# Shinzef/BlenderRayTracer

Hardware: AMD Instinct MI355X
Metric: Msamples/s (pixels×spp/s) at 1/2/4/8 MI355X; % HBM roofline; RMS vs JS ref (higher is better)
Workload: dtype f64; 1 GPU; config3_rtow_1920x1080_512spp; scene=rtow.json, width=1920, height=1080, spp=512, max_depth=5, primitives=486, accel=auto, parallelism=1 GPU

## Files before the change

__graft_entry__.py:

```python
import os
import sys

ROOT = os.path.dirname(os.path.abspath(__file__))
if ROOT not in sys.path:
    sys.path.insert(0, ROOT)


def build() -> None:
    from blenderraytracer_amd import build as b
    b.build_lib(force=True)
    b.build_cli(force=True)
    b.build_napi(force=True)
    from oracle import binding
    binding.build()
    sys.path.insert(0, os.path.join(ROOT, "tests"))
    import hostcheck_binding
    hostcheck_binding.build()
    hostcheck_binding.lib(("RT_HOST_COUNTERS=1",))
    import texcheck_binding
    texcheck_binding.build()
    import lightcheck_binding
    lightcheck_binding.build()
    import guidedcheck_binding
    guidedcheck_binding.build()
    import neecheck_binding
    for mutation in (0, 1, 2):
        neecheck_binding.build(mutation)
    import blenderraytracer_amd
    from blenderraytracer_amd import capi
    capi.load_library()


def smoke() -> None:
    import numpy as np

    from blenderraytracer_amd import capi
    from blenderraytracer_amd.renderer import GpuRayTracer
    from blenderraytracer_amd.scene import load_scene_json
    from oracle import binding

    rt = GpuRayTracer(64, 48, seed=7, device=0, precision=capi.RT_PREC_F64)
    assert rt.load_from_json(load_scene_json("sample_scene.json"))
    rt.update_render_settings({"maxBounces": 4, "samples": 4})
    r = rt.render(want=("mean", "segments"))
    o = binding.render(rt.packed(), rt.settings())
    assert np.array_equal(r["segments"], o["segments"]), "segment counts differ from the oracle"
    err = np.max(np.abs(r["mean"] - o["mean"]))
    assert err <= 1e-12, f"GPU vs oracle max abs diff {err}"
    assert np.array_equal(r["rgba8"], o["rgba8"])
    print(f"smoke ok: 64x48x4spp sample_scene, {rt.last_stats.kernel_ms:.3f} ms kernel, max|diff| {err:.1e}")
    rt.close()
    rt = GpuRayTracer(48, 27, seed=7, device=0, precision=capi.RT_PREC_F64)
    assert rt.load_from_json(load_scene_json("rtow.json"))
    rt.update_render_settings({"maxBounces": 5, "samples": 4})
    lib = capi.load_library()
    assert lib.rt_scene_walk(rt.scene_handle(), capi.RT_PREC_F64, capi.RT_ACCEL_AUTO) == 2, "RTOW should walk the grid"
    r = rt.render(want=("mean", "segments"))
    o = binding.render(rt.packed(), rt.settings())
    assert np.array_equal(r["segments"], o["segments"]), "RTOW segment counts differ from the oracle"
    err = np.max(np.abs(r["mean"] - o["mean"]))
# ... 11 lines not shown
```

blenderraytracer_amd/csrc/pt_core.h:

```cpp
#pragma once
#include <hip/hip_runtime.h>
#include <math.h>
#include <stdint.h>
#include <string.h>
#include "js_math.h"

#define RT_HD __host__ __device__ __forceinline__
#ifndef RT_COLD_BG
#define RT_COLD_BG 1
#endif
#if RT_COLD_BG && defined(__HIP_DEVICE_COMPILE__)
#define RT_COLD __attribute__((noinline))
#else
#define RT_COLD
#endif
#define RT_COLD_HD __host__ __device__ RT_COLD

namespace rt {

template <class R> RT_HD R js_pow(R x, R y) {
    if constexpr (sizeof(R) == 8) return jsm::pow(x, y);
    else return pow(x, y);
}
template <class R> RT_HD R js_exp(R x) {
// ... 107 lines not shown
    if (div_rcp_on<R>() && min3abs(a) >= xmin && l >= smin && l <= smax)
        return {div_rcp_1(a.x, l, y), div_rcp_1(a.y, l, y), div_rcp_1(a.z, l, y)};
    return vdiv(a, l);
}
template <class R> RT_HD V3<R> normalize(V3<R> a) {
    R l = sqrt(a.x * a.x + a.y * a.y + a.z * a.z);
#if RT_DIV_RCP
    return l > (R)0 ? vdiv_rcp_unit(a, l, (R)1 / l) : mk<R>(0, 0, 0);
#else
    return l > (R)0 ? vdiv(a, l) : mk<R>(0, 0, 0);
#endif
}
template <class R> RT_HD V3<R> reflect(V3<R> a, V3<R> n) {
    return a - n * ((R)2 * dot(a, n));
}

enum RunKind : int { RUN_SPHERES = 0, RUN_PLANES = 1, RUN_BOXES = 2, RUN_TRIANGLES = 3, RUN_MESH = 4 };
struct Run { int kind, begin, end, mat; };

template <class R> struct SphereRec { R cx, cy, cz, r2; };
struct SphereFilter { float cx, cy, cz, r2p; };
#ifndef RT_FILTER_MARGIN
#define RT_FILTER_MARGIN (-17)
#endif
constexpr double filter_margin() {
    double v = 1.0;
    for (int k = 0; k > RT_FILTER_MARGIN; --k) v *= 0.5;
    return v;
}
template <class R> struct PlaneRec { R px, py, pz, nx, ny, nz; };
template <class R> struct BoxRec { R mnx, mny, mnz, mxx, mxy, mxz; };
template <class R> struct TriRec { R v0x, v0y, v0z, e1x, e1y, e1z, e2x, e2y, e2z, nx, ny, nz; };
template <class R> struct MatRec { int type, pad; R c[3]; R p; };
template <class R> struct SphereLeaf { SphereFilter f; SphereRec<R> s; int id, obj, mat, pad; };
template <> struct SphereLeaf<float> { SphereRec<float> s; int id, obj, mat, pad; };
template <class R> struct TriGeom { R v0x, v0y, v0z, e1x, e1y, e1z, e2x, e2y, e2z; };
template <class R> struct alignas(16) TriLeaf { TriGeom<R> t; int id, obj; };
struct alignas(16) TriFilter { float v0[3], e1[3], e2[3], n[3]; };

struct BvhNode { float lo[3]; int skip; float hi[3]; int fc; };
struct Bvh2Node { float lo[3][2]; float hi[3][2]; int child[2]; int pad[2]; };
#ifndef RT_BVH_STACK
#define RT_BVH_STACK 24
#endif

enum TexType : int { TEX_CHECKER = 0, TEX_NOISE = 1, TEX_MARBLE = 2, TEX_WOOD = 3 };
template <class R> struct TexRec { int type, perm; R scale; R odd[3], even[3]; };
template <class R> struct TexView { const TexRec<R>* recs; const int* perms; const int* mat_tex; int num, num_perms; };
enum LightType : int { LIGHT_POINT = 0, LIGHT_DIRECTIONAL = 1 };
template <class R> struct LightRec { int type, pad; R v[3]; R color[3]; R intensity; };
template <class R> struct LightView { const LightRec<R>* recs; int num, pad; };
enum EmitterKind : int { EMIT_SPHERE = 0, EMIT_TRI = 1 };
template <class R> struct EmitterRec { int kind, idx; R g[12]; R le[3]; R area; };
template <class R> struct EmitterView { const EmitterRec<R>* recs; const int* sphere_listed; const R* tri_area; int num, pad; };

template <class R>
struct SceneView {
    const Run* runs;
    int num_runs;
    int num_prims;
    const SphereRec<R>* spheres;
    const SphereFilter* sphere_filter;
    int num_spheres;
    const R* sphere_r;
    const R* sphere_inv_r;
    const PlaneRec<R>* planes;
    const BoxRec<R>* boxes;
// ... 139 lines not shown
#if RT_FAST_RCP && defined(__HIP_DEVICE_COMPILE__)
    return __builtin_amdgcn_rcpf(x);
#else
    return 1.0f / x;
#endif
}
RT_HD float rt_rsqrt_approx(float x) {
#if RT_FAST_RCP && defined(__HIP_DEVICE_COMPILE__)
    return __builtin_amdgcn_rsqf(x);
#else
    return 1.0f / sqrtf(x);
#endif
}

struct FilterRay { float ox, oy, oz, dx, dy, dz, delta; };

template <class R>
RT_HD FilterRay make_filter_ray(V3<R> o, V3<R> d) {
    FilterRay f;
    f.ox = (float)o.x; f.oy = (float)o.y; f.oz = (float)o.z;
    const float dx = (float)d.x, dy = (float)d.y, dz = (float)d.z;
    const float inv = rt_rsqrt_approx(dx * dx + dy * dy + dz * dz);
    f.dx = dx * inv; f.dy = dy * inv; f.dz = dz * inv;
    f.delta = (f.ox * f.ox + f.oy * f.oy + f.oz * f.oz) * ((float)(2.0 * filter_margin()) * (1.0f + 0x1p-20f));
    return f;
}

RT_HD bool sphere_filter_pass(const SphereFilter& s, const FilterRay& r) {
    RT_HCOUNT(HC_FILTER_TESTS, 1);
    const float ocx = r.ox - s.cx, ocy = r.oy - s.cy, ocz = r.oz - s.cz;
    const float hb = __builtin_fmaf(ocx, r.dx, __builtin_fmaf(ocy, r.dy, ocz * r.dz));
    const float cc = __builtin_fmaf(ocx, ocx, __builtin_fmaf(ocy, ocy, __builtin_fmaf(ocz, ocz, -(s.r2p + r.delta))));
    return !(__builtin_fmaf(hb, hb, -cc) < 0.0f);
}

enum Feat : int { F_PLANES = 1, F_BOXES = 2, F_TRIS = 4, F_BGALL = 8, F_CAMALL = 16, F_ALL = 31,
                  F_TEX = 32,
                  F_LIGHT = 64,
                  F_NEE = 128 };

template <class R, int FEAT = F_ALL>
RT_HD Closest<R> closest_hit_runs(const SceneView<R>& sc, V3<R> o, V3<R> d) {
    const R tmin = (R)0.001;
    Closest<R> b{(R)INFINITY, HIT_NONE, 0, 0};
    const R a = dot(d, d);
    for (int r = 0; r < sc.num_runs; ++r) {
        const Run run = sc.runs[r];
        if (run.kind == RUN_SPHERES) {
            if constexpr (sizeof(R) == 8) {
                const FilterRay fr = make_filter_ray(o, d);
RT_UNROLL(RT_SPHERE_UNROLL)
                for (int i = run.begin; i < run.end; ++i) {
                    if (!sphere_filter_pass(sc.sphere_filter[i], fr)) continue;
                    sphere_test_f64(sc, o, d, a, tmin, i, b);
                }
                continue;
            }
#pragma unroll 2
            for (int i = run.begin; i < run.end; ++i) sphere_test_f64(sc, o, d, a, tmin, i, b);
        } else if ((FEAT & F_PLANES) != 0 && run.kind == RUN_PLANES) {
            for (int i = run.begin; i < run.end; ++i) {
                const PlaneRec<R> p = sc.planes[i];
                R denom = p.nx * d.x + p.ny * d.y + p.nz * d.z;
                if (fabs(denom) < (R)1e-6) continue;
                R t = ((p.px - o.x) * p.nx + (p.py - o.y) * p.ny + (p.pz - o.z) * p.nz) / denom;
                if (t < tmin || t > b.t) continue;
// ... 439 lines not shown
    const BvhRay br = make_bvh_ray(o, d);
    float tl = bvh_tlimit(b.t);
    if (sc.num_sphere_nodes > 0 || sc.num_big_spheres > 0) {
        const R a = dot(d, d);
        FilterRay fr{};
        if constexpr (sizeof(R) == 8) fr = make_filter_ray(o, d);
        if (sc.num_big_spheres > 0) sphere_records(sc.big_spheres, 0, sc.num_big_spheres, o, d, a, fr, tmin, b, tl, w, true);
        auto leaf = [&](int fc) { sphere_leaf(sc, fc, o, d, a, fr, tmin, b, tl, w); };
        if (sc.num_sphere_nodes > 0)
            bvh_walk<WIDE, LDSN ? 1 : 0>(sc.sphere_nodes, sc.num_sphere_nodes, sc.sphere_wide, br, tl, stk, w, leaf);
    }
    if (TRI && sc.num_tri_nodes > 0 && !skip_tri) {
        if constexpr (sizeof(R) == 8 && RT_TRI_FILTER != 0) {
            const TriRay tr = make_tri_ray(o, d);
            auto leaf = [&](int fc) { tri_leaf_filtered(sc, fc, tr, o, d, tmin, b, tl, w); };
            bvh_walk<WIDE, TLDS ? 2 : 0>(sc.tri_nodes, sc.num_tri_nodes, sc.tri_wide, br, tl, stk, w, leaf);
        } else {
            auto leaf = [&](int fc) { tri_leaf(sc, fc, o, d, tmin, b, tl, w); };
            bvh_walk<WIDE, TLDS ? 2 : 0>(sc.tri_nodes, sc.num_tri_nodes, sc.tri_wide, br, tl, stk, w, leaf);
        }
    }
    return b;
}

#ifndef RT_GRID_UNIFORM
#define RT_GRID_UNIFORM 2
#endif
#ifndef RT_GRID_DIV
#define RT_GRID_DIV 0
#endif
#ifndef RT_GRID_COMPACT
#define RT_GRID_COMPACT 1
#endif
template <class R>
RT_HD void sphere_records_lds(const rt_u4* lrec, const SphereLeaf<R>* recs, int first, int end, V3<R> o, V3<R> d,
                              R a, const FilterRay& fr, R tmin, Closest<R>& b, float& tl, Work& w, R ya = (R)0,
                              int origin = -1) {
    RT_COUNT(w.spheres += end - first);
    if constexpr (sizeof(R) == 8 && RT_GRID_COMPACT != 0) {
        for (int base = first; base < end; base += 32) {
            const int n = end - base < 32 ? end - base : 32;
            uint32_t pass = 0;
            for (int i = 0; i < n; ++i) {
                const rt_u4 q = lrec[base + i];
                SphereFilter f;
                memcpy(&f, &q, sizeof f);
                if (sphere_filter_pass(f, fr)) pass |= 1u << i;
            }
            while (pass) {
                const int k = base + __builtin_ctz(pass);
                pass &= pass - 1;
                const SphereRec<R> s = recs[k].s;
                const int id = recs[k].id, obj = recs[k].obj, mat = recs[k].mat;
                R t;
                if (!sphere_candidate(s, o, d, a, tmin, t, RT_ORIGIN_LEAVE && id == origin, ya)) continue;
                if (better(t, obj, id, b)) {
                    RT_HCOUNT(HC_ACCEPT, 1);
                    b = Closest<R>{t, HIT_SPHERE, id, mat, obj};
                    tl = bvh_tlimit(b.t);
                }
            }
        }
        return;
    }
    for (int k = first; k < end; ++k) {
        SphereRec<R> s;
        int id, obj, mat;
        if constexpr (sizeof(R) == 8) {
            const rt_u4 q = lrec[k];
            SphereFilter f;
            memcpy(&f, &q, sizeof f);
            if (!sphere_filter_pass(f, fr)) continue;
            s = recs[k].s;
            id = recs[k].id; obj = recs[k].obj; mat = recs[k].mat;
        } else {
            const rt_u4 q0 = lrec[2 * k], q1 = lrec[2 * k + 1];
            memcpy(&s, &q0, sizeof s);
            id = (int)q1.x; obj = (int)q1.y; mat = (int)q1.z;
        }
        R t;
        if (!sphere_candidate(s, o, d, a, tmin, t, false, ya)) continue;
        if (better(t, obj, id, b)) {
            RT_HCOUNT(HC_ACCEPT, 1);
            b = Closest<R>{t, HIT_SPHERE, id, mat, obj};
            tl = bvh_tlimit(b.t);
        }
    }
}

template <class R>
RT_HD size_t grid_lds_rec_bytes(const SceneView<R>& sc) { return (size_t)sc.num_grid_recs * (sizeof(R) == 8 ? 16 : 32); }
template <class R>
RT_HD size_t grid_lds_bytes(const SceneView<R>& sc) {
    return grid_lds_rec_bytes(sc) + 4 * (size_t)(sc.num_grid_cells + 1);
}
template <class R>
RT_HD void copy_grid_lds(const SceneView<R>& sc, rt_u4* grec, int* gcell, int t, int threads) {
    const rt_u4* g = reinterpret_cast<const rt_u4*>(sc.grid_leaf);
    for (int k = t; k < sc.num_grid_recs; k += threads) {
        if constexpr (sizeof(R) == 8) grec[k] = g[4 * k];
        else { grec[2 * k] = g[2 * k]; grec[2 * k + 1] = g[2 * k + 1]; }
    }
    for (int k = t; k <= sc.num_grid_cells; k += threads) gcell[k] = sc.grid_cell[k];
}

struct GridRefs { const int* n; const float *lo, *hi, *cs, *ics; float far; };

template <class R, bool LDSG = false, int FEAT = F_ALL, bool LOCAL = false>
RT_HD Closest<R> closest_hit_grid(const SceneView<R>& sc, V3<R> o, V3<R> d, Work& w, const BvhStack& stk, int origin = -1) {
    const R tmin = (R)0.001;
    Closest<R> b{(R)INFINITY, HIT_NONE, 0, 0, -1};
    brute_planes_boxes<R, FEAT>(sc, o, d, tmin, b);
    float tl = bvh_tlimit(b.t);
    const R a = dot(d, d), ya = root_rcp(a);
    FilterRay fr{};
    if constexpr (sizeof(R) == 8) fr = make_filter_ray(o, d);
    if (sc.num_big_spheres > 0) sphere_records(sc.big_spheres, 0, sc.num_big_spheres, o, d, a, fr, tmin, b, tl, w, true, ya);
    if (sc.num_grid_cells <= 0) return b;
    const GridRefs gp{sc.grid_n, sc.grid_lo, sc.grid_hi, sc.grid_cs, sc.grid_ics, sc.grid_far};
    auto at = [](const auto* a, int k) {
        if constexpr (LOCAL) return k == 0 ? a[0] : (k == 1 ? a[1] : a[2]);
        else return a[k];
    };
    const float of[3] = {(float)o.x, (float)o.y, (float)o.z};
    const float df[3] = {(float)d.x, (float)d.y, (float)d.z};
    if (!(fmaxf(fabsf(of[0]), fmaxf(fabsf(of[1]), fabsf(of[2]))) <= gp.far)) {
        sphere_records(sc.grid_leaf, 0, sc.grid_cell[sc.num_grid_cells], o, d, a, fr, tmin, b, tl, w);
        return b;
    }
    float inv[3], t0 = 0.0f, t1 = tl;
    for (int k = 0; k < 3; ++k) {
        float v = rt_rcp_approx(df[k]);
        if (!(fabsf(v) <= 0x1p126f)) v = copysignf(0x1p126f, df[k]);
        inv[k] = v;
        const float ta = (gp.lo[k] - of[k]) * v, tb = (gp.hi[k] - of[k]) * v;
        t0 = fmaxf(t0, fminf(ta, tb));
        t1 = fminf(t1, fmaxf(ta, tb));
    }
    if (!(t0 <= t1)) return b;
    int cell[3], step[3];
    float tmax[3];
    for (int k = 0; k < 3; ++k) {
        const float p = of[k] + t0 * df[k];
        const bool by_div = RT_GRID_DIV == 1 || (RT_GRID_DIV == 0 && sizeof(R) == 8);
        int c = by_div ? (int)floorf((p - gp.lo[k]) / gp.cs[k])
                       : (int)floorf((p - gp.lo[k]) * gp.ics[k]);
        c = c < 0 ? 0 : (c >= gp.n[k] ? gp.n[k] - 1 : c);
        cell[k] = c;
        step[k] = df[k] > 0.0f ? 1 : (df[k] < 0.0f ? -1 : 0);
        tmax[k] = step[k] == 0 ? INFINITY
                               : (gp.lo[k] + (float)(c + (step[k] > 0)) * gp.cs[k] - of[k]) * inv[k];
    }
    for (;;) {
        RT_COUNT(++w.nodes);
        const int ci = cell[0] + gp.n[0] * (cell[1] + gp.n[1] * cell[2]);
        if constexpr (LDSG) {
            sphere_records_lds(stk.grec, sc.grid_leaf, stk.gcell[ci], stk.gcell[ci + 1], o, d, a, fr, tmin, b, tl, w, ya, origin);
        } else {
#if RT_GRID_UNIFORM && defined(__HIP_DEVICE_COMPILE__)
        const int first = __builtin_amdgcn_readfirstlane(ci);
        if ((RT_GRID_UNIFORM == 1 || sizeof(R) == 4) && __ballot(ci != first) == 0)
            sphere_records(sc.grid_leaf, sc.grid_cell[first], sc.grid_cell[first + 1], o, d, a, fr, tmin, b, tl, w);
        else
#endif
        sphere_records(sc.grid_leaf, sc.grid_cell[ci], sc.grid_cell[ci + 1], o, d, a, fr, tmin, b, tl, w);
        }
        const int ax = tmax[0] <= tmax[1] ? (tmax[0] <= tmax[2] ? 0 : 2) : (tmax[1] <= tmax[2] ? 1 : 2);
        const float tx = tmax[ax];
        if (b.t < (R)tx || !(tx < INFINITY)) break;
        const int nc = cell[ax] + step[ax];
        if (nc < 0 || nc >= at(gp.n, ax)) break;
        cell[ax] = nc;
        tmax[ax] = (at(gp.lo, ax) + (float)(nc + (step[ax] > 0)) * at(gp.cs, ax) - of[ax]) * inv[ax];
    }
    return b;
}

enum Accel : int { ACC_BRUTE = 0, ACC_BRUTE_LEAN = 1, ACC_BVH = 2, ACC_BVH_STACK = 3, ACC_BVH_SPHERES = 4, ACC_BVH_SPHERES_LDS = 5,
                   ACC_GRID = 6, ACC_GRID_LDS = 7, ACC_BVH_TRI_LDS = 8, ACC_GRID_LDS_LEAN = 9,
                   ACC_BVH_STACK_LEAN = 10, ACC_BRUTE_TEX = 11, ACC_BVH_STACK_TEX = 12,
                   ACC_BRUTE_LIT = 13, ACC_BVH_STACK_LIT = 14, ACC_BRUTE_NEE = 15, ACC_BVH_STACK_NEE = 16 };
template <int ACC> constexpr int walk_of() {
    return ACC == ACC_BRUTE_TEX || ACC == ACC_BRUTE_LIT || ACC == ACC_BRUTE_NEE ? ACC_BRUTE
         : ACC == ACC_BVH_STACK_TEX || ACC == ACC_BVH_STACK_LIT || ACC == ACC_BVH_STACK_NEE ? ACC_BVH_STACK : ACC;
}
template <int ACC> constexpr int feat_of() {
    return ACC == ACC_GRID_LDS_LEAN ? 0 : ACC == ACC_BVH_STACK_LEAN ? (F_PLANES | F_TRIS)
         : ACC == ACC_BRUTE_LEAN ? F_PLANES : ACC == ACC_BRUTE_TEX || ACC == ACC_BVH_STACK_TEX ? (F_ALL | F_TEX)
         : ACC == ACC_BRUTE_LIT || ACC == ACC_BVH_STACK_LIT ? (F_ALL | F_TEX | F_LIGHT)
         : ACC == ACC_BRUTE_NEE || ACC == ACC_BVH_STACK_NEE ? (F_ALL | F_TEX | F_LIGHT | F_NEE) : F_ALL;
}

#ifndef RT_SC_RELOAD
#define RT_SC_RELOAD 2
#endif
template <class R, int ACC> constexpr bool sc_reload() {
    return sizeof(R) == 8 && (((RT_SC_RELOAD & 1) && ACC == ACC_BVH_STACK_LEAN) ||
                              ((RT_SC_RELOAD & 2) && ACC == ACC_GRID_LDS_LEAN) || ((RT_SC_RELOAD & 4) && ACC == ACC_BRUTE_LEAN));
}
template <class R, int ACC, bool LOCAL = false>
RT_HD Closest<R> closest_hit_acc(const SceneView<R>& sc, V3<R> o, V3<R> d, Work& w, BvhStack stk, bool skip_tri = false,
                                 int origin = -1) {
#if defined(__HIP_DEVICE_COMPILE__)
    if constexpr (!LOCAL && sc_reload<R, ACC>()) {
        typedef const __attribute__((address_space(4))) SceneView<R>* SvPtr;
        SvPtr p = (SvPtr)__builtin_amdgcn_kernarg_segment_ptr();
        asm volatile("" : "+s"(p));
        const SceneView<R> scl = *p;
        return closest_hit_acc<R, ACC, true>(scl, o, d, w, stk, skip_tri, origin);
    }
#endif
    if constexpr (walk_of<ACC>() != ACC) return closest_hit_acc<R, walk_of<ACC>(), LOCAL>(sc, o, d, w, stk, skip_tri, origin);
    else if constexpr (ACC == ACC_BVH) return closest_hit_bvh<R, false>(sc, o, d, w, stk, skip_tri);
    else if constexpr (ACC == ACC_BVH_STACK) return closest_hit_bvh<R, true>(sc, o, d, w, stk, skip_tri);
    else if constexpr (ACC == ACC_BVH_SPHERES) return closest_hit_bvh<R, true, false>(sc, o, d, w, stk);
    else if constexpr (ACC == ACC_BVH_SPHERES_LDS) return closest_hit_bvh<R, true, false, true>(sc, o, d, w, stk);
    else if constexpr (ACC == ACC_GRID) return closest_hit_grid<R>(sc, o, d, w, stk);
    else if constexpr (ACC == ACC_GRID_LDS) return closest_hit_grid<R, true>(sc, o, d, w, stk);
    else if constexpr (ACC == ACC_GRID_LDS_LEAN) return closest_hit_grid<R, true, feat_of<ACC>(), LOCAL>(sc, o, d, w, stk, origin);
    else if constexpr (ACC == ACC_BVH_STACK_LEAN)
        return closest_hit_bvh<R, true, true, false, false, feat_of<ACC>()>(sc, o, d, w, stk, skip_tri);
    else if constexpr (ACC == ACC_BVH_TRI_LDS) return closest_hit_bvh<R, true, true, false, true>(sc, o, d, w, stk);
    else return closest_hit_runs<R, feat_of<ACC>()>(sc, o, d);
}

template <class R, int FEAT = F_ALL>
RT_HD bool occluded_runs(const SceneView<R>& sc, V3<R> o, V3<R> d, R tmax) {
    const R tmin = (R)0.001;
    Closest<R> b{tmax, HIT_NONE, 0, 0};
    const R a = dot(d, d);
    for (int r = 0; r < sc.num_runs; ++r) {
        const Run run = sc.runs[r];
        if (run.kind == RUN_SPHERES) {
            if constexpr (sizeof(R) == 8) {
                const FilterRay fr = make_filter_ray(o, d);
                for (int i = run.begin; i < run.end; ++i) {
                    if (!sphere_filter_pass(sc.sphere_filter[i], fr)) continue;
                    sphere_test_f64(sc, o, d, a, tmin, i, b);
                    if (b.kind != HIT_NONE) return true;
                }
                continue;
            }
            for (int i = run.begin; i < run.end; ++i) {
                sphere_test_f64(sc, o, d, a, tmin, i, b);
                if (b.kind != HIT_NONE) return true;
            }
        } else if ((FEAT & F_PLANES) != 0 && run.kind == RUN_PLANES) {
            for (int i = run.begin; i < run.end; ++i) {
                const PlaneRec<R> p = sc.planes[i];
                R denom = p.nx * d.x + p.ny * d.y + p.nz * d.z;
                if (fabs(denom) < (R)1e-6) continue;
                R t = ((p.px - o.x) * p.nx + (p.py - o.y) * p.ny + (p.pz - o.z) * p.nz) / denom;
// ... 355 lines not shown
```

blenderraytracer_amd/csrc/pt_guided.hip:

```cpp
#include <algorithm>

#include "pt_guided.h"
#include "kernel_select.h"

namespace rt {

namespace {

__device__ __forceinline__ void stage_wide_nodes(const Bvh2Node* src, int n, rt_u4* box, rt_u2* kid, int t) {
    for (int k = t; k < n; k += 64) {
        const rt_u4* g = reinterpret_cast<const rt_u4*>(src + k);
        const rt_u4 q3 = g[3];
        box[3 * k] = g[0];
        box[3 * k + 1] = g[1];
        box[3 * k + 2] = g[2];
        kid[k] = rt_u2{q3.x, q3.y};
    }
}

template <class R, int ACC>
__device__ __forceinline__ BvhStack stage_walk_lds(const SceneView<R>& sc, unsigned char* lds_dyn) {
    BvhStack stk{nullptr, 0};
    if constexpr (ACC == ACC_GRID_LDS || ACC == ACC_GRID_LDS_LEAN) {
        rt_u4* grec = reinterpret_cast<rt_u4*>(lds_dyn);
        int* gcell = reinterpret_cast<int*>(lds_dyn + grid_lds_rec_bytes(sc));
        copy_grid_lds(sc, grec, gcell, threadIdx.x, 64);
        stk.gcell = gcell;
        stk.grec = grec;
    } else {
        constexpr bool TOP = ACC == ACC_BVH_TRI_LDS;
        const WideLds l{TOP ? sc.tri_lds_nodes : sc.num_sphere_wide, min(sc.stack_entries, RT_BVH_STACK)};
        rt_u4* box = reinterpret_cast<rt_u4*>(lds_dyn + l.boxes());
        rt_u2* kid = reinterpret_cast<rt_u2*>(lds_dyn + l.kids());
        stage_wide_nodes(TOP ? sc.tri_wide : sc.sphere_wide, l.n, box, kid, threadIdx.x);
        stk = BvhStack{reinterpret_cast<int*>(lds_dyn + l.stacks()) + threadIdx.x, 64, box, kid};
        if constexpr (TOP) stk.ntop = l.n;
    }
    return stk;
}

}

template <class R, int ACC>
__global__ __launch_bounds__(64) void aov_kernel(const SceneView<R> sc, const AovFrame f, float* __restrict__ guides,
                                                 int* __restrict__ kind_out, int* __restrict__ idx_out) {
    BvhStack stk{nullptr, 0};
    if constexpr (lds_form(ACC)) {
        extern __shared__ __attribute__((aligned(16))) unsigned char lds_dyn[];
        stk = stage_walk_lds<R, ACC>(sc, lds_dyn);
        __syncthreads();
    } else {
        __shared__ int stack[RT_BVH_STACK * 64];
        stk = BvhStack{stack + threadIdx.x, 64};
    }
    const size_t r = (size_t)blockIdx.x * 64 + threadIdx.x;
    if (r >= (size_t)f.cw * (size_t)f.ch) return;
    const int cx = (int)(r % (size_t)f.cw), cy = (int)(r / (size_t)f.cw);
    float g[8];
    const AovHit h = aov_pixel<R, ACC>(sc, f.width, f.height, f.x0 + cx, f.height - 1 - (f.y0 + cy), stk, g);
// ... 60 lines not shown
```

blenderraytracer_amd/csrc/pt_trace.hip:

```cpp
#include <algorithm>
#include <atomic>
#include <chrono>
#include <cmath>
#include <cstdlib>
#include <cstring>
#include <mutex>
#include <thread>
#include <type_traits>
#include <vector>

#include "pt_launch.h"
#include "kernel_select.h"
#include "pool_order.h"
#include "queue_slots.h"

namespace rt {

template <class R>
struct TraceArgs {
    SceneView<R> sc;
    ImageParams im;
    Counters c;
};
static_assert(offsetof(TraceArgs<double>, sc) == 0 && offsetof(TraceArgs<float>, sc) == 0, "sc first");
// ... 96 lines not shown
        }
        stk.stride = 64;
    }
    const int lane = threadIdx.x;
    const Tile t = tile_of(im, blockIdx.x);
    const int cx = t.x0 + (lane & 7), cy = t.y0 + (lane >> 3);
    const bool valid = cx < im.cw && cy < im.ch;
    const size_t q = (size_t)cy * im.cw + cx;
    double acc[3] = {0, 0, 0};
    if (valid) { acc[0] = args.c.sum[3 * q]; acc[1] = args.c.sum[3 * q + 1]; acc[2] = args.c.sum[3 * q + 2]; }
    const PixelResult r = trace_pixel<R, COUNT, ACC>(args.sc, im, cx, cy, valid ? im.s_end : im.s_begin, acc, stk);
    if (valid) {
        args.c.sum[3 * q] = acc[0]; args.c.sum[3 * q + 1] = acc[1]; args.c.sum[3 * q + 2] = acc[2];
        if (COUNT) {
            if (args.c.segs) args.c.segs[q] += r.segments;
            if (args.c.draws) args.c.draws[q] += r.draws;
        }
    }
    add_totals<ACC>(args.c, r, lane);
}

#ifndef RT_PARK
#define RT_PARK 0
#endif
constexpr int kParkDoubles = 3, kParkInts = 6;
template <class R, int ACC>
constexpr bool parks() { return RT_PARK != 0 && sizeof(R) == 8 && uses_stack<ACC>(); }

#ifndef RT_DEFER_REGEN
#define RT_DEFER_REGEN 16
#endif
#ifndef RT_DEFER_REGEN_TRI
#define RT_DEFER_REGEN_TRI 48
#endif
template <class R>
__device__ __forceinline__ int defer_regen(const SceneView<R>& sc) {
    return sc.num_tri_nodes > 0 ? RT_DEFER_REGEN_TRI : RT_DEFER_REGEN;
}

template <class R, bool COUNT, int ACC, bool CANCEL>
__global__ __launch_bounds__(64, (waves_per_simd<R, ACC>()))
void trace_pool_kernel(const TraceArgs<R> args, double* __restrict__ part, const int tiles, const int chunk) {
    const ImageParams& im = args.im;
    const SceneView<R>& sc = args.sc;
    constexpr bool PARK = parks<R, ACC>();
    BvhStack stk{nullptr, 0};
    double* park_d = nullptr;
    uint32_t* park_i = nullptr;
    if constexpr (PARK) {
        extern __shared__ double park_dyn[];
        park_d = park_dyn + threadIdx.x;
        park_i = reinterpret_cast<uint32_t*>(park_dyn + kParkDoubles * 64) + threadIdx.x;
        stk.base = reinterpret_cast<int*>(park_dyn + kParkDoubles * 64) + kParkInts * 64 + threadIdx.x;
        stk.stride = 64;
    } else if constexpr (uses_stack<ACC>()) {
        if constexpr (sizeof(R) == 8 && !dyn_stack<R, ACC>()) {
            __shared__ int bvh_stack[RT_BVH_STACK * 64];
            stk.base = bvh_stack + threadIdx.x;
        } else {
            extern __shared__ int bvh_stack_dyn[];
            stk.base = bvh_stack_dyn + threadIdx.x;
        }
        stk.stride = 64;
    }
    __shared__ double acc[3 * 64];
    const int lane = threadIdx.x;
// ... 121 lines not shown
            args.c.sum[3 * qq + 2] += acc[128 + lane];
        }
    }
    if (args.c.batch_count) {
        if (im.bands) {
            const int bb = band_of_tile(im, tile);
            item_done(args.c, bb, band_items(im, bb), 1, lane);
        } else {
            item_done(args.c, cr.b, (uint32_t)(im.batch_chunks * tiles), im.batch_ways, lane);
        }
    }
    add_totals<ACC>(args.c, res, lane);
}

template <class R, bool COUNT, int ACC>
__device__ __forceinline__ void pool_item(const TraceArgs<R>& args, double* __restrict__ part, const int tiles,
                                          const int chunk, const unsigned pos, double* acc, BvhStack stk,
                                          PixelResult& res, const int lane, const MatRec<R>* lmats = nullptr) {
    const ImageParams& im = args.im;
    const SceneView<R>& sc = args.sc;
    const unsigned item = item_at(im, pos, tiles);
    const int tile = item % tiles;
    const ChunkRange cr = chunk_range(im, (int)(item / tiles), chunk);
    const Tile tl = tile_of(im, tile);
    const int vw = tl.vw, nv = tl.nv;
    const int sb = cr.sb, se = cr.se;
    const uint32_t total = (uint32_t)nv * (uint32_t)max(0, se - sb);
    int i = 0, j = 0, s = 0, depth = 0;
    uint32_t m = 0, pkey = 0, isegs = 0;
    size_t q = 0;
    Rng<R> g;
    V3<R> o, d, T;
    auto begin_item = [&](const uint32_t k) {
        uint32_t sr;
        if (nv == 64) { m = k & 63; sr = k >> 6; }
        else { sr = k / (uint32_t)nv; m = k - sr * (uint32_t)nv; }
        const int px = tl.x0 + (int)(m % (uint32_t)vw), py = tl.y0 + (int)(m / (uint32_t)vw);
        const int row = im.y0 + py;
        i = im.x0 + px;
        j = im.height - 1 - row;
        pkey = pixel_key(im.seedm, (uint32_t)row * (uint32_t)im.width + (uint32_t)i);
        q = (size_t)py * im.cw + px;
        s = sb + (int)sr;
        T = mk<R>(1, 1, 1);
        depth = im.max_depth;
        isegs = 0;
        start_sample<R, sizeof(R) == 4 || (RT_CAM_RELOAD_LEAN64 != 0 && ACC == ACC_GRID_LDS_LEAN), feat_of<ACC>()>(sc, im, i, j, pkey, s, g, o, d);
    };
    uint32_t next = 64;
    const int defer_k = defer_regen(sc);
    bool live = (uint32_t)lane < total;
    if (live) begin_item((uint32_t)lane);
    bool waiting = false;
    int origin = -1;
    while (live) {
        const uint64_t t0 = RT_TICK();
        if (!waiting) {
            const Closest<R> c = closest_hit_acc<R, ACC>(sc, o, d, res.work, stk, false, origin);
            const uint64_t t1 = RT_TICK();
            if (RT_PROFILE) res.cyc[0] += t1 - t0;
            ++res.segments;
            ++isegs;
            V3<R> L;
            waiting = shade_segment<R, feat_of<ACC>()>(sc, c, o, d, T, depth, g, L, lmats);
            if constexpr (RT_ORIGIN_LEAVE && sizeof(R) == 8 && ACC == ACC_GRID_LDS_LEAN)
                origin = !waiting && c.kind == HIT_SPHERE ? c.idx : -1;
            if (RT_PROFILE) res.cyc[1] += RT_TICK() - t1;
            if (waiting) {
                if (COUNT) {
                    if (args.c.segs) atomicAdd(args.c.segs + q, isegs);
// ... 52 lines not shown
    acc[128 + lane] = 0;
    __builtin_amdgcn_fence(__ATOMIC_SEQ_CST, "wavefront");
    __builtin_amdgcn_wave_barrier();
}

#if !RT_ONEWAVE_TU
constexpr int kPoolQueues = 1024;
__device__ uint32_t g_pool_queue[2 * kPoolQueues];

__device__ __forceinline__ void copy_wide_lds(const Bvh2Node* src, int n, rt_u4* box, rt_u2* kid, int t, int threads) {
    for (int k = t; k < n; k += threads) {
        const rt_u4* g = reinterpret_cast<const rt_u4*>(src + k);
        const rt_u4 q3 = g[3];
        box[3 * k] = g[0];
        box[3 * k + 1] = g[1];
        box[3 * k + 2] = g[2];
        kid[k] = rt_u2{q3.x, q3.y};
    }
}

template <class R, bool COUNT, int ACC>
__global__ __launch_bounds__((64 * lds_waves<R, ACC>()), (waves_per_simd<R, ACC>()))
void trace_pool_lds_kernel(const TraceArgs<R> args, double* __restrict__ part, const int tiles, const int chunk,
                           const int items, const int qi) {
    constexpr int W = lds_waves<R, ACC>();
    const SceneView<R>& sc = args.sc;
    extern __shared__ __attribute__((aligned(16))) unsigned char lds_dyn[];
    __shared__ double acc_all[W * 3 * 64];
    const int wave = threadIdx.x >> 6, lane = threadIdx.x & 63;
    BvhStack stk{nullptr, 0};
    if constexpr (ACC == ACC_GRID_LDS || ACC == ACC_GRID_LDS_LEAN) {
        rt_u4* grec = reinterpret_cast<rt_u4*>(lds_dyn);
        int* gcell = reinterpret_cast<int*>(lds_dyn + grid_lds_rec_bytes(sc));
        copy_grid_lds(sc, grec, gcell, threadIdx.x, 64 * W);
        stk.gcell = gcell;
        stk.grec = grec;
    } else if constexpr (ACC == ACC_BVH_TRI_LDS) {
        const int n = sc.tri_lds_nodes, entries = min(sc.stack_entries, RT_BVH_STACK);
        rt_u4* box = reinterpret_cast<rt_u4*>(lds_dyn);
        rt_u2* kid = reinterpret_cast<rt_u2*>(lds_dyn + 48 * n);
        int* stacks = reinterpret_cast<int*>(lds_dyn + 56 * n);
        copy_wide_lds(sc.tri_wide, n, box, kid, threadIdx.x, 64 * W);
        stk = BvhStack{stacks + wave * entries * 64 + lane, 64, box, kid};
        stk.ntop = n;
    } else {
        const int n = sc.num_sphere_wide, entries = min(sc.stack_entries, RT_BVH_STACK);
        rt_u4* box = reinterpret_cast<rt_u4*>(lds_dyn);
        rt_u2* kid = reinterpret_cast<rt_u2*>(lds_dyn + 48 * n);
        int* stacks = reinterpret_cast<int*>(lds_dyn + 56 * n);
        copy_wide_lds(sc.sphere_wide, n, box, kid, threadIdx.x, 64 * W);
        stk = BvhStack{stacks + wave * entries * 64 + lane, 64, box, kid};
    }
    double* acc = acc_all + wave * 3 * 64;
    acc[lane] = 0;
    acc[64 + lane] = 0;
    acc[128 + lane] = 0;
    const MatRec<R>* lmats = nullptr;
#if RT_MAT_LDS
    if constexpr (ACC == ACC_GRID_LDS || ACC == ACC_GRID_LDS_LEAN) {
        MatRec<R>* mm = reinterpret_cast<MatRec<R>*>(lds_dyn + ((grid_lds_bytes(sc) + 15) & ~(size_t)15));
        for (int k = threadIdx.x; k < sc.num_mats; k += 64 * W) mm[k] = sc.mats[k];
        lmats = mm;
    }
#endif
    __syncthreads();
    uint32_t* queue = g_pool_queue + 2 * qi;
    PixelResult res{0, 0, {0, 0, 0}, {0, 0, 0}};
// ... 531 lines not shown
    if (im0.cw <= 0 || im0.ch <= 0 || im0.s_end <= im0.s_begin || bands <= 0) return hipSuccess;
    const PoolPlan p = pool_plan(im0.cw, im0.ch, im0.s_end - im0.s_begin, sc.num_tri_nodes > 0, im0.pool_chunk);
    if (plan) *plan = p;
    if (!part || !c.batch_count || !c.batch_flag || part_bytes < p.part_bytes || bands > (im0.ch + 7) / 8)
        return hipErrorInvalidValue;
    if ((long long)p.tiles * p.chunks > 0x7FFFFFFFLL) return hipErrorInvalidConfiguration;
    ImageParams im = im0;
    im.pool_chunk = p.chunk;
    im.bands = bands;
    im.band_chunks = p.chunks;
    return launch_partials(sc, im, c, bvh, p, part, stream);
}
template hipError_t launch_trace_bands<double>(const SceneView<double>&, const ImageParams&, const Counters&, bool, int,
                                               double*, size_t, PoolPlan*, hipStream_t);
template hipError_t launch_trace_bands<float>(const SceneView<float>&, const ImageParams&, const Counters&, bool, int,
                                              double*, size_t, PoolPlan*, hipStream_t);

hipError_t launch_reduce(const ImageParams& im, double* sum, const double* part, bool tri_bvh, hipStream_t stream,
                         const ReduceGate* gate) {
    if (im.cw <= 0 || im.ch <= 0 || im.s_end <= im.s_begin) return hipSuccess;
    const PoolPlan p = pool_plan(im.cw, im.ch, im.s_end - im.s_begin, tri_bvh, im.pool_chunk);
    if (gate) hipLaunchKernelGGL(reduce_gate_kernel, dim3(1), dim3(64), 0, stream, *gate);
    hipLaunchKernelGGL(reduce_kernel, dim3((unsigned)p.tiles), dim3(64), 0, stream, im, sum, part, p.tiles, p.chunks,
                       (const uint32_t*)(gate ? gate->skip : nullptr));
    return hipGetLastError();
}

template <class R, int ACC>
__device__ __forceinline__ BvhStack stage_lds_wave(const SceneView<R>& sc, unsigned char* lds_dyn) {
    BvhStack stk{nullptr, 0};
    if constexpr (ACC == ACC_GRID_LDS || ACC == ACC_GRID_LDS_LEAN) {
        rt_u4* grec = reinterpret_cast<rt_u4*>(lds_dyn);
        int* gcell = reinterpret_cast<int*>(lds_dyn + grid_lds_rec_bytes(sc));
        copy_grid_lds(sc, grec, gcell, threadIdx.x, 64);
        stk.gcell = gcell;
        stk.grec = grec;
    } else {
        constexpr bool TOP = ACC == ACC_BVH_TRI_LDS;
        const WideLds l{TOP ? sc.tri_lds_nodes : sc.num_sphere_wide, min(sc.stack_entries, RT_BVH_STACK)};
        rt_u4* box = reinterpret_cast<rt_u4*>(lds_dyn + l.boxes());
        rt_u2* kid = reinterpret_cast<rt_u2*>(lds_dyn + l.kids());
        copy_wide_lds(TOP ? sc.tri_wide : sc.sphere_wide, l.n, box, kid, threadIdx.x, 64);
        stk = BvhStack{reinterpret_cast<int*>(lds_dyn + l.stacks()) + threadIdx.x, 64, box, kid};
        if constexpr (TOP) stk.ntop = l.n;
    }
    return stk;
}
template <class R, int ACC>
__global__ __launch_bounds__(64) void closest_hits_kernel(const SceneView<R> sc, const double* __restrict__ rays,
                                                          const size_t n, double* __restrict__ t_out,
                                                          int* __restrict__ kind_out, int* __restrict__ idx_out) {
    BvhStack stk{nullptr, 0};
    if constexpr (lds_form(ACC)) {
        extern __shared__ __attribute__((aligned(16))) unsigned char lds_dyn[];
        stk = stage_lds_wave<R, ACC>(sc, lds_dyn);
        __syncthreads();
    } else {
        __shared__ int stack[RT_BVH_STACK * 64];
        stk = BvhStack{stack + threadIdx.x, 64};
    }
    const size_t r = (size_t)blockIdx.x * 64 + threadIdx.x;
    if (r >= n) return;
    const double* q = rays + 6 * r;
    const V3<R> o = mk<R>((R)q[0], (R)q[1], (R)q[2]), d = mk<R>((R)q[3], (R)q[4], (R)q[5]);
    Work w{0, 0, 0, 0, 0, 0};
    const Closest<R> c = closest_hit_acc<R, ACC>(sc, o, d, w, stk);
    t_out[r] = c.kind == HIT_NONE ? (double)INFINITY : (double)c.t;
// ... 324 lines not shown
```

blenderraytracer_amd/csrc/scene_pack.h:

```cpp
#pragma once
#include <algorithm>
#include <cmath>
#include <cstdio>
#include <cstdlib>
#include <cstring>
#include <string>
#include <thread>
#include <vector>

#include "../../include/rt_hip.h"
#include "pt_core.h"

namespace rt {

struct HostScene {
    std::vector<Run> runs;
    std::vector<double> spheres, sphere_r, planes, boxes, tris;
    std::vector<int> sphere_mat, plane_mat, box_mat, tri_mat;
    std::vector<int> sphere_obj, plane_obj, box_obj, tri_obj;
    std::vector<double> tri_verts;
    std::vector<BvhNode> sphere_bvh, tri_bvh;
    std::vector<int> sphere_bvh_prims, tri_bvh_prims;
    std::vector<int> big_spheres;
    std::vector<Bvh2Node> sphere_wide, tri_wide;
// ... 779 lines not shown
            for (int k = 0; k < 3; ++k) { r.v[k] = (R)l.v[k]; r.color[k] = (R)l.color[k]; }
            r.intensity = (R)l.intensity;
            out.light_recs[i] = r;
        }
    }
    if (!hs.emit_idx.empty()) {
        if (out.mat_tex.empty()) out.mat_tex.assign((size_t)std::max(1, d.num_materials), -1);
        out.sphere_listed.assign(std::max<size_t>(1, out.spheres.size()), 0);
        out.tri_area.assign(std::max<size_t>(1, out.tris.size()), (R)0);
        out.emitter_recs.resize(hs.emit_idx.size());
        for (size_t e = 0; e < hs.emit_idx.size(); ++e) {
            EmitterRec<R> r{};
            r.kind = hs.emit_kind[e];
            r.idx = hs.emit_idx[e];
            int mat;
            if (r.kind == EMIT_SPHERE) {
                const SphereRec<R>& s = out.spheres[r.idx];
                r.g[0] = s.cx; r.g[1] = s.cy; r.g[2] = s.cz; r.g[3] = s.r2;
                out.sphere_listed[r.idx] = 1;
                mat = hs.sphere_mat[r.idx];
            } else {
                const double* t = &hs.tris[12 * (size_t)r.idx];
                for (int k = 0; k < 12; ++k) r.g[k] = (R)t[k];
                r.area = (R)tri_area64(t);
                out.tri_area[r.idx] = r.area;
                mat = hs.tri_mat[r.idx];
            }
            for (int k = 0; k < 3; ++k) r.le[k] = out.mats[mat].c[k];
            out.emitter_recs[e] = r;
        }
    }
    auto leaf = [&](int id) {
        SphereLeaf<R> L{};
        if constexpr (sizeof(R) == 8) L.f = out.sphere_filter[id];
        L.s = out.spheres[id];
        L.id = id;
        L.obj = hs.sphere_obj[id];
        L.mat = hs.sphere_mat[id];
        return L;
    };
    for (int id : hs.sphere_bvh_prims) out.bvh_sphere_leaf.push_back(leaf(id));
    for (int id : hs.big_spheres) out.big_sphere_leaf.push_back(leaf(id));
    for (int id : hs.grid_ids) out.grid_leaf.push_back(leaf(id));
    for (int id : hs.tri_bvh_prims) {
        const TriRec<R>& r = out.tris[id];
        out.bvh_tri_leaf.push_back(TriLeaf<R>{{r.v0x, r.v0y, r.v0z, r.e1x, r.e1y, r.e1z, r.e2x, r.e2y, r.e2z},
                                              id, hs.tri_obj[id]});
        if constexpr (sizeof(R) == 8) out.tri_filter.push_back(make_tri_filter(&hs.tris[12 * (size_t)id]));
    }
}

template <class R>
void fill_view_constants(SceneView<R>& v, const HostScene& hs, const rt_scene_desc& d) {
    v.num_runs = (int)hs.runs.size();
    v.num_spheres = (int)hs.sphere_r.size();
    v.num_prims = hs.num_prims;
    v.num_planes = (int)hs.plane_mat.size();
    v.num_mats = d.num_materials;
    v.num_tex = scene_textured(d) ? d.num_textures : 0;
    v.num_lights = d.num_lights;
    v.num_emitters = (int)hs.emit_idx.size();
    v.num_boxes = (int)hs.box_mat.size();
    v.num_sphere_nodes = (int)hs.sphere_bvh.size();
    v.num_tri_nodes = (int)hs.tri_bvh.size();
    v.num_sphere_wide = (int)hs.sphere_wide.size();
    v.num_tri_wide = (int)hs.tri_wide.size();
    v.num_big_spheres = (int)hs.big_spheres.size();
// ... 105 lines not shown
```

Measured before the change: 11190 Msamples/s.

## Precompute per-sphere filter constant and remap grid tiles to 8x8 blocks

Rewrites the float sphere pre-filter so that per-sphere constants (|c|^2 - r^2 with a conservative margin) are computed on the host and stored in the LDS record's last word. Per-ray terms are hoisted into an expanded filter ray, which cuts the per-sphere FMA count in the grid LDS lean path. It also maps 64-lane tiles to 8x8 pixel blocks instead of row strips, aiming for better ray coherence. The risks are that the conservative bounds of the rearranged filter could differ slightly, and that a different pixel-to-lane mapping could change ordering.

```diff
diff --git a/__graft_entry__.py b/__graft_entry__.py
--- a/__graft_entry__.py
+++ b/__graft_entry__.py
@@ -26,6 +26,8 @@
     import neecheck_binding
     for mutation in (0, 1, 2):
         neecheck_binding.build(mutation)
+    import filterxcheck_binding
+    filterxcheck_binding.build()
     import blenderraytracer_amd
     from blenderraytracer_amd import capi
     capi.load_library()
diff --git a/blenderraytracer_amd/csrc/pt_core.h b/blenderraytracer_amd/csrc/pt_core.h
--- a/blenderraytracer_amd/csrc/pt_core.h
+++ b/blenderraytracer_amd/csrc/pt_core.h
@@ -163,7 +163,7 @@
 template <class R> struct BoxRec { R mnx, mny, mnz, mxx, mxy, mxz; };
 template <class R> struct TriRec { R v0x, v0y, v0z, e1x, e1y, e1z, e2x, e2y, e2z, nx, ny, nz; };
 template <class R> struct MatRec { int type, pad; R c[3]; R p; };
-template <class R> struct SphereLeaf { SphereFilter f; SphereRec<R> s; int id, obj, mat, pad; };
+template <class R> struct SphereLeaf { SphereFilter f; SphereRec<R> s; int id, obj, mat; float kx; };
 template <> struct SphereLeaf<float> { SphereRec<float> s; int id, obj, mat, pad; };
 template <class R> struct TriGeom { R v0x, v0y, v0z, e1x, e1y, e1z, e2x, e2y, e2z; };
 template <class R> struct alignas(16) TriLeaf { TriGeom<R> t; int id, obj; };
@@ -369,6 +369,35 @@
     const float hb = __builtin_fmaf(ocx, r.dx, __builtin_fmaf(ocy, r.dy, ocz * r.dz));
     const float cc = __builtin_fmaf(ocx, ocx, __builtin_fmaf(ocy, ocy, __builtin_fmaf(ocz, ocz, -(s.r2p + r.delta))));
     return !(__builtin_fmaf(hb, hb, -cc) < 0.0f);
+}
+
+#ifndef RT_FILTER_X
+#define RT_FILTER_X 1
+#endif
+struct SphereFilterX { float cx, cy, cz, k; };
+struct FilterRayX { float ox2, oy2, oz2, dx, dy, dz, A, B; };
+
+inline float filter_x_k(const SphereFilter& f) {
+    const double c2 = ((double)f.cx * f.cx + (double)f.cy * f.cy) + (double)f.cz * f.cz;
+    const double kd = ((double)f.r2p - c2) + 0x1p-40 * ((double)f.r2p + c2);
+    if (!(fabs(kd) <= 3.4028234663852886e38)) return INFINITY;
+    float k = (float)kd;
+    if ((double)k < kd) k = nextafterf(k, INFINITY);
+    return k;
+}
+RT_HD FilterRayX make_filter_ray_x(const FilterRay& f) {
+    FilterRayX x;
+    x.ox2 = f.ox + f.ox; x.oy2 = f.oy + f.oy; x.oz2 = f.oz + f.oz;
+    x.dx = f.dx; x.dy = f.dy; x.dz = f.dz;
+    x.A = __builtin_fmaf(f.ox, f.dx, __builtin_fmaf(f.oy, f.dy, f.oz * f.dz));
+    x.B = f.delta - (f.ox * f.ox + f.oy * f.oy + f.oz * f.oz);
+    return x;
+}
+RT_HD bool sphere_filter_x_pass(const SphereFilterX& s, const FilterRayX& r) {
+    RT_HCOUNT(HC_FILTER_TESTS, 1);
+    const float h = __builtin_fmaf(-s.cx, r.dx, __builtin_fmaf(-s.cy, r.dy, __builtin_fmaf(-s.cz, r.dz, r.A)));
+    const float e = __builtin_fmaf(r.ox2, s.cx, __builtin_fmaf(r.oy2, s.cy, __builtin_fmaf(r.oz2, s.cz, s.k + r.B)));
+    return !(__builtin_fmaf(h, h, e) < 0.0f);
 }
 
 enum Feat : int { F_PLANES = 1, F_BOXES = 2, F_TRIS = 4, F_BGALL = 8, F_CAMALL = 16, F_ALL = 31,
@@ -874,9 +903,19 @@
 #ifndef RT_GRID_COMPACT
 #define RT_GRID_COMPACT 1
 #endif
-template <class R>
+RT_HD bool lds_filter_pass(const rt_u4& q, const FilterRay& fr) {
+    SphereFilter f;
+    memcpy(&f, &q, sizeof f);
+    return sphere_filter_pass(f, fr);
+}
+RT_HD bool lds_filter_pass(const rt_u4& q, const FilterRayX& fr) {
+    SphereFilterX f;
+    memcpy(&f, &q, sizeof f);
+    return sphere_filter_x_pass(f, fr);
+}
+template <class R, class FR>
 RT_HD void sphere_records_lds(const rt_u4* lrec, const SphereLeaf<R>* recs, int first, int end, V3<R> o, V3<R> d,
-                              R a, const FilterRay& fr, R tmin, Closest<R>& b, float& tl, Work& w, R ya = (R)0,
+                              R a, const FR& fr, R tmin, Closest<R>& b, float& tl, Work& w, R ya = (R)0,
                               int origin = -1) {
     RT_COUNT(w.spheres += end - first);
     if constexpr (sizeof(R) == 8 && RT_GRID_COMPACT != 0) {
@@ -885,9 +924,7 @@
             uint32_t pass = 0;
             for (int i = 0; i < n; ++i) {
                 const rt_u4 q = lrec[base + i];
-                SphereFilter f;
-                memcpy(&f, &q, sizeof f);
-                if (sphere_filter_pass(f, fr)) pass |= 1u << i;
+                if (lds_filter_pass(q, fr)) pass |= 1u << i;
             }
             while (pass) {
                 const int k = base + __builtin_ctz(pass);
@@ -910,9 +947,7 @@
         int id, obj, mat;
         if constexpr (sizeof(R) == 8) {
             const rt_u4 q = lrec[k];
-            SphereFilter f;
-            memcpy(&f, &q, sizeof f);
-            if (!sphere_filter_pass(f, fr)) continue;
+            if (!lds_filter_pass(q, fr)) continue;
             s = recs[k].s;
             id = recs[k].id; obj = recs[k].obj; mat = recs[k].mat;
         } else {
@@ -936,11 +971,16 @@
 RT_HD size_t grid_lds_bytes(const SceneView<R>& sc) {
     return grid_lds_rec_bytes(sc) + 4 * (size_t)(sc.num_grid_cells + 1);
 }
-template <class R>
+template <class R, bool XF = false>
 RT_HD void copy_grid_lds(const SceneView<R>& sc, rt_u4* grec, int* gcell, int t, int threads) {
     const rt_u4* g = reinterpret_cast<const rt_u4*>(sc.grid_leaf);
     for (int k = t; k < sc.num_grid_recs; k += threads) {
-        if constexpr (sizeof(R) == 8) grec[k] = g[4 * k];
+        if constexpr (sizeof(R) == 8 && XF) {
+            rt_u4 q = g[4 * k];
+            q.w = g[4 * k + 3].w;
+            grec[k] = q;
+        }
+        else if constexpr (sizeof(R) == 8) grec[k] = g[4 * k];
         else { grec[2 * k] = g[2 * k]; grec[2 * k + 1] = g[2 * k + 1]; }
     }
     for (int k = t; k <= sc.num_grid_cells; k += threads) gcell[k] = sc.grid_cell[k];
@@ -948,7 +988,7 @@
 
 struct GridRefs { const int* n; const float *lo, *hi, *cs, *ics; float far; };
 
-template <class R, bool LDSG = false, int FEAT = F_ALL, bool LOCAL = false>
+template <class R, bool LDSG = false, int FEAT = F_ALL, bool LOCAL = false, bool XF = false>
 RT_HD Closest<R> closest_hit_grid(const SceneView<R>& sc, V3<R> o, V3<R> d, Work& w, const BvhStack& stk, int origin = -1) {
     const R tmin = (R)0.001;
     Closest<R> b{(R)INFINITY, HIT_NONE, 0, 0, -1};
@@ -957,6 +997,9 @@
     const R a = dot(d, d), ya = root_rcp(a);
     FilterRay fr{};
     if constexpr (sizeof(R) == 8) fr = make_filter_ray(o, d);
+    static_assert(!XF || (sizeof(R) == 8 && LDSG), "the expanded filter reads binary64 LDS records");
+    FilterRayX fx{};
+    if constexpr (XF) fx = make_filter_ray_x(fr);
     if (sc.num_big_spheres > 0) sphere_records(sc.big_spheres, 0, sc.num_big_spheres, o, d, a, fr, tmin, b, tl, w, true, ya);
     if (sc.num_grid_cells <= 0) return b;
     const GridRefs gp{sc.grid_n, sc.grid_lo, sc.grid_hi, sc.grid_cs, sc.grid_ics, sc.grid_far};
@@ -996,7 +1039,9 @@
     for (;;) {
         RT_COUNT(++w.nodes);
         const int ci = cell[0] + gp.n[0] * (cell[1] + gp.n[1] * cell[2]);
-        if constexpr (LDSG) {
+        if constexpr (LDSG && XF) {
+            sphere_records_lds(stk.grec, sc.grid_leaf, stk.gcell[ci], stk.gcell[ci + 1], o, d, a, fx, tmin, b, tl, w, ya, origin);
+        } else if constexpr (LDSG) {
             sphere_records_lds(stk.grec, sc.grid_leaf, stk.gcell[ci], stk.gcell[ci + 1], o, d, a, fr, tmin, b, tl, w, ya, origin);
         } else {
 #if RT_GRID_UNIFORM && defined(__HIP_DEVICE_COMPILE__)
@@ -1031,6 +1076,10 @@
          : ACC == ACC_BRUTE_LEAN ? F_PLANES : ACC == ACC_BRUTE_TEX || ACC == ACC_BVH_STACK_TEX ? (F_ALL | F_TEX)
          : ACC == ACC_BRUTE_LIT || ACC == ACC_BVH_STACK_LIT ? (F_ALL | F_TEX | F_LIGHT)
          : ACC == ACC_BRUTE_NEE || ACC == ACC_BVH_STACK_NEE ? (F_ALL | F_TEX | F_LIGHT | F_NEE) : F_ALL;
+}
+
+template <class R, int ACC> constexpr bool grid_filter_x() {
+    return RT_FILTER_X != 0 && sizeof(R) == 8 && ACC == ACC_GRID_LDS_LEAN;
 }
 
 #ifndef RT_SC_RELOAD
@@ -1059,7 +1108,7 @@
     else if constexpr (ACC == ACC_BVH_SPHERES_LDS) return closest_hit_bvh<R, true, false, true>(sc, o, d, w, stk);
     else if constexpr (ACC == ACC_GRID) return closest_hit_grid<R>(sc, o, d, w, stk);
     else if constexpr (ACC == ACC_GRID_LDS) return closest_hit_grid<R, true>(sc, o, d, w, stk);
-    else if constexpr (ACC == ACC_GRID_LDS_LEAN) return closest_hit_grid<R, true, feat_of<ACC>(), LOCAL>(sc, o, d, w, stk, origin);
+    else if constexpr (ACC == ACC_GRID_LDS_LEAN) return closest_hit_grid<R, true, feat_of<ACC>(), LOCAL, grid_filter_x<R, ACC>()>(sc, o, d, w, stk, origin);
     else if constexpr (ACC == ACC_BVH_STACK_LEAN)
         return closest_hit_bvh<R, true, true, false, false, feat_of<ACC>()>(sc, o, d, w, stk, skip_tri);
     else if constexpr (ACC == ACC_BVH_TRI_LDS) return closest_hit_bvh<R, true, true, false, true>(sc, o, d, w, stk);
diff --git a/blenderraytracer_amd/csrc/pt_guided.hip b/blenderraytracer_amd/csrc/pt_guided.hip
--- a/blenderraytracer_amd/csrc/pt_guided.hip
+++ b/blenderraytracer_amd/csrc/pt_guided.hip
@@ -24,7 +24,7 @@
     if constexpr (ACC == ACC_GRID_LDS || ACC == ACC_GRID_LDS_LEAN) {
         rt_u4* grec = reinterpret_cast<rt_u4*>(lds_dyn);
         int* gcell = reinterpret_cast<int*>(lds_dyn + grid_lds_rec_bytes(sc));
-        copy_grid_lds(sc, grec, gcell, threadIdx.x, 64);
+        copy_grid_lds<R, grid_filter_x<R, ACC>()>(sc, grec, gcell, threadIdx.x, 64);
         stk.gcell = gcell;
         stk.grec = grec;
     } else {
diff --git a/blenderraytracer_amd/csrc/pt_trace.hip b/blenderraytracer_amd/csrc/pt_trace.hip
--- a/blenderraytracer_amd/csrc/pt_trace.hip
+++ b/blenderraytracer_amd/csrc/pt_trace.hip
@@ -152,6 +152,9 @@
 #endif
 #ifndef RT_DEFER_REGEN_TRI
 #define RT_DEFER_REGEN_TRI 48
+#endif
+#ifndef RT_TILE_SHIFT
+#define RT_TILE_SHIFT 1
 #endif
 template <class R>
 __device__ __forceinline__ int defer_regen(const SceneView<R>& sc) {
@@ -339,10 +342,12 @@
     Rng<R> g;
     V3<R> o, d, T;
     auto begin_item = [&](const uint32_t k) {
-        uint32_t sr;
+        uint32_t sr, mx, my;
         if (nv == 64) { m = k & 63; sr = k >> 6; }
         else { sr = k / (uint32_t)nv; m = k - sr * (uint32_t)nv; }
-        const int px = tl.x0 + (int)(m % (uint32_t)vw), py = tl.y0 + (int)(m / (uint32_t)vw);
+        if (RT_TILE_SHIFT && sizeof(R) == 8 && ACC == ACC_GRID_LDS_LEAN && nv == 64) { mx = m & 7; my = m >> 3; }
+        else { mx = m % (uint32_t)vw; my = m / (uint32_t)vw; }
+        const int px = tl.x0 + (int)mx, py = tl.y0 + (int)my;
         const int row = im.y0 + py;
         i = im.x0 + px;
         j = im.height - 1 - row;
@@ -461,7 +466,7 @@
     if constexpr (ACC == ACC_GRID_LDS || ACC == ACC_GRID_LDS_LEAN) {
         rt_u4* grec = reinterpret_cast<rt_u4*>(lds_dyn);
         int* gcell = reinterpret_cast<int*>(lds_dyn + grid_lds_rec_bytes(sc));
-        copy_grid_lds(sc, grec, gcell, threadIdx.x, 64 * W);
+        copy_grid_lds<R, grid_filter_x<R, ACC>()>(sc, grec, gcell, threadIdx.x, 64 * W);
         stk.gcell = gcell;
         stk.grec = grec;
     } else if constexpr (ACC == ACC_BVH_TRI_LDS) {
@@ -1059,7 +1064,7 @@
     if constexpr (ACC == ACC_GRID_LDS || ACC == ACC_GRID_LDS_LEAN) {
         rt_u4* grec = reinterpret_cast<rt_u4*>(lds_dyn);
         int* gcell = reinterpret_cast<int*>(lds_dyn + grid_lds_rec_bytes(sc));
-        copy_grid_lds(sc, grec, gcell, threadIdx.x, 64);
+        copy_grid_lds<R, grid_filter_x<R, ACC>()>(sc, grec, gcell, threadIdx.x, 64);
         stk.gcell = gcell;
         stk.grec = grec;
     } else {
diff --git a/blenderraytracer_amd/csrc/scene_pack.h b/blenderraytracer_amd/csrc/scene_pack.h
--- a/blenderraytracer_amd/csrc/scene_pack.h
+++ b/blenderraytracer_amd/csrc/scene_pack.h
@@ -835,7 +835,7 @@
     }
     auto leaf = [&](int id) {
         SphereLeaf<R> L{};
-        if constexpr (sizeof(R) == 8) L.f = out.sphere_filter[id];
+        if constexpr (sizeof(R) == 8) { L.f = out.sphere_filter[id]; L.kx = filter_x_k(L.f); }
         L.s = out.spheres[id];
         L.id = id;
         L.obj = hs.sphere_obj[id];
```

Result: faster. 11310 Msamples/s (median of 6 runs) (+1.1%).
